# RKWin93/E2E-MAPPO-for-MT-FJSP

Measured on AMD Instinct MI355X. Metric: env-steps/sec (batched J6M6E2), higher is better.
Workload: dtype f64 (environment) / f32 (encoder: f32 storage and accumulation; 128x128 products on the 16-bit matrix cores from split f32 operands, f32-accurate: DESIGN.md §4)

## Files before the change

__graft_entry__.py:

```python
#!/usr/bin/env python3
import os
import sys

ROOT = os.path.dirname(os.path.abspath(__file__))
if ROOT not in sys.path:
    sys.path.insert(0, ROOT)


def build() -> None:
    from importlib import import_module
    import mtfjsp_amd
    _build = import_module("e2e-mappo-for-mt-fjsp_amd._build")
    lib = _build.build(force=True, verbose=True)
    capi = import_module("e2e-mappo-for-mt-fjsp_amd.capi")
    capi.lib()
    print("variant:", _build.build_variant("funcs", ["-DMTFJSP_BODY_FUNCS=3"]))
    from oracle import env_oracle
    print("oracle:", env_oracle.build(force=True))
    print("built", lib)


def smoke() -> None:
    import numpy as np
    import torch
    from importlib import import_module
    import mtfjsp_amd
    assert torch.cuda.is_available(), "smoke() needs cuda:0"
    batch_env = import_module("e2e-mappo-for-mt-fjsp_amd.batch_env")
    inst = import_module("e2e-mappo-for-mt-fjsp_amd.instances")
    from oracle.env_oracle import OracleBatch
    J, M, E, B = 6, 6, 2, 8
    T = J * M
    t, p, tt, edge = inst.generate_instances(B, J, M, E, seed=0)
    import random
    random.seed(0)
    w3 = inst.random_weights(B)
    env = batch_env.DeviceBatchEnv(J, M, E, B, obs_dtype="f64")
    env.load_instances(t, p, tt, edge=edge)
    env.scaler_init()
    env.reset(w3)
    orc = OracleBatch(t, p, tt, edge)
    orc.scaler_init()
    orc.reset(w3)
    a = torch.zeros(B, dtype=torch.int32, device=env.device); m = torch.zeros_like(a); j = torch.zeros_like(a)
    for s in range(T):
        env.random_actions(7, s, a, m, j)
        env.step(a, m)
        info, raw, _ = orc.step(a.cpu().numpy(), m.cpu().numpy())
        cand, mask = orc.job_mask_update(j.cpu().numpy())
        o = orc.observe()
        assert np.array_equal(env.info.cpu().numpy(), info), f"step {s}: rewards differ"
        assert np.array_equal(env.tasks_fea.cpu().numpy(), o["tfea"]), f"step {s}: tasks_fea differ"
        assert np.array_equal(env.dense_adj().cpu().numpy(), o["adj"]), f"step {s}: adj differ"
        assert np.array_equal(env.m_fea2.cpu().numpy(), o["mfea2"])
        assert np.array_equal(env.candidate.cpu().numpy(), cand) and np.array_equal(env.job_mask.cpu().numpy(), mask)
    assert bool(env.info[:, 1].all())
    _smoke_encoder()
    print("smoke OK: HIP env == oracle on", B, "instances x", T, "steps")


def _smoke_encoder() -> None:
    try:
        from importlib import import_module
        enc = import_module("e2e-mappo-for-mt-fjsp_amd.encoder")
    except ImportError:
        return
    if hasattr(enc, "smoke"):
        enc.smoke()


if __name__ == "__main__":
    cmd = sys.argv[1] if len(sys.argv) > 1 else "build"
    {"build": build, "smoke": smoke}[cmd]()
```

e2e-mappo-for-mt-fjsp_amd/csrc/mtfjsp_encoder.hip:

```cpp
#include <hip/hip_runtime.h>
#include <math.h>
#include <stdint.h>
#include <stdio.h>
#include <stdlib.h>
#include <string.h>
#include <algorithm>
#include <map>
#include <stdexcept>
#include <string>
#include <vector>

#include "../../include/mtfjsp.h"


#include "mtfjsp_enc_shared.h"

enum { PRO_PLAIN = 0, PRO_BNRELU = 1, PRO_AGG = 2, PRO_GIN0 = 3, PRO_GIN0BN = 4 };
enum { EPI_PLAIN = 0, EPI_STATS = 1, EPI_TANH = 2 };

struct GemmArgs {
    const float *in;
    int N;
    const float *Wt;
    const void *Wx6;
// ... 1279 lines not shown
__device__ __forceinline__ float pick_uniform(int b, uint64_t seed, uint64_t counter)
{
    uint32_t c[4] = {(uint32_t)b, (uint32_t)counter, (uint32_t)(counter >> 32), 0x73616d70u};
    philox4x32(c, (uint32_t)seed, (uint32_t)(seed >> 32));
    return (float)(c[0] >> 8) * (1.0f / 16777216.0f);
}
__device__ __forceinline__ int pick_action_u(const float *p, int n, int greedy, float u)
{
    int pick = 0;
    if (greedy) {
        float best = p[0];
        for (int i = 1; i < n; i++) if (p[i] > best) { best = p[i]; pick = i; }
    } else {
        float tot = 0.f;
        for (int i = 0; i < n; i++) tot += p[i];
        float acc = 0.f;
        const float thr = u * tot;
        pick = -1;
        int last = 0;
        for (int i = 0; i < n; i++) {
            if (p[i] > 0.f) {
                last = i;
                acc += p[i];
                if (pick < 0 && thr < acc) pick = i;
            }
        }
        if (pick < 0) pick = last;
    }
    return pick;
}
__device__ __forceinline__ int pick_action(const float *p, int n, int b, int greedy, uint64_t seed, uint64_t counter)
{
    int pick = 0;
    if (greedy) {
        float best = p[0];
        for (int i = 1; i < n; i++) if (p[i] > best) { best = p[i]; pick = i; }
    } else {
        uint32_t c[4] = {(uint32_t)b, (uint32_t)counter, (uint32_t)(counter >> 32), 0x73616d70u};
        philox4x32(c, (uint32_t)seed, (uint32_t)(seed >> 32));
        const float u = (float)(c[0] >> 8) * (1.0f / 16777216.0f);
        float tot = 0.f;
        for (int i = 0; i < n; i++) tot += p[i];
        float acc = 0.f;
        const float thr = u * tot;
        pick = -1;
        int last = 0;
        for (int i = 0; i < n; i++) {
            if (p[i] > 0.f) {
                last = i;
                acc += p[i];
                if (pick < 0 && thr < acc) pick = i;
            }
        }
        if (pick < 0) pick = last;
    }
    return pick;
}

struct HeadArgs {
    int B, R;
    int hg;
    const float *X;
    const float *pooled, *other;
    const float *W0i;
    const float *b0, *W1i, *b1, *w2, *b2;
    const float *Wc0i, *bc0, *Wc1i, *bc1, *wc2, *bc2;
    const void *W0x, *W1x, *Wc0x, *Wc1x;
    float sW0, sW1, sWc0, sWc1;
    const uint8_t *mask;
    float scale;
    float *prob, *value;
    const double *xbn_stats; const float *xbn_gamma, *xbn_beta; double xbn_inv_rows; float *pooled_out;
    const int *xgather; int xT, xrelu;
    int sample_mode; unsigned long long seed, counter; int *idx_out; float *logp_out; const int *gather_from; int *gathered_out;
    mtfjsp_mfea1_ctx_t mf; int mf_on;
    double *zero_stats; int zero_count;
    double *zero_stats2; int zero_count2;
    unsigned long long *stamps;
    unsigned *range_flag;
};
#define HG 16
#define HCH 6
#define HX_NPART 32

__global__ __launch_bounds__(512) void k_heads(HeadArgs A)
{
    extern __shared__ __align__(16) unsigned char smem[];
    float *s_x = reinterpret_cast<float *>(smem);
    float *s_s = s_x + HCH * 16 * LDA16;
    float *s_p = s_s + HCH * 16 * LDA16;
    float *s_o = s_p + 16 * LDA16;
    float *s_c1 = s_o + 16 * LDA16;
    float *s_c2 = s_c1 + 16 * LDA16;
    float *s_u = s_c2 + 16 * LDA16;
    float *s_part = s_u + HG * HD;
    float *s_score = s_part + 8 * HCH * 16;
    float *s_wc2 = s_score + HG * 64;
    unsigned char *s_mask = reinterpret_cast<unsigned char *>(s_wc2 + 2 * HD);
    const int tid = threadIdx.x, wave = tid >> 6, lane = tid & 63;
    const int m = lane & 15, q = lane >> 4;
    const int col = 16 * wave + m;
#ifdef MTFJSP_STAMP
    unsigned long long ph[8] = {0, 0, 0, 0, 0, 0, 0, 0}, t_last;
    asm volatile("s_memtime %0\n\ts_waitcnt lgkmcnt(0)" : "=s"(t_last)::"memory");
#endif
    const int R = A.R;
    const unsigned invR = (unsigned)((0x100000000ull + (unsigned)R - 1) / (unsigned)R);
#define WCOL(dst, Wi)                                                                              \
    do {                                                                                           \
        const float4 *w_ = reinterpret_cast<const float4 *>(Wi) + (size_t)wave * 8 * 64 + lane;    \
        _Pragma("unroll") for (int g_ = 0; g_ < 8; g_++) {                                         \
            const float4 v_ = w_[g_ * 64];                                                         \
            dst[4 * g_] = v_.x; dst[4 * g_ + 1] = v_.y; dst[4 * g_ + 2] = v_.z; dst[4 * g_ + 3] = v_.w; \
        }                                                                                          \
    } while (0)
#define TILE2(acc0, acc1, t0p, t1p, bw)                                                                          \
    do {                                                                                                         \
        _Pragma("unroll") for (int s_ = 0; s_ < 32; s_++) {                                                      \
            acc0 = __builtin_amdgcn_mfma_f32_16x16x4f32((t0p)[4 * s_], bw[s_], acc0, 0, 0, 0);                   \
            acc1 = __builtin_amdgcn_mfma_f32_16x16x4f32((t1p)[4 * s_], bw[s_], acc1, 0, 0, 0);                   \
        }                                                                                                        \
        MFMA_SETTLE2(acc0, acc1);                                                                                \
    } while (0)
    const int sr = tid >> 5, sc4 = (tid & 31) * 4;
    const int aoff = m * LDA16 + q;
    const float b0c = A.b0[col], bc0c = A.bc0[col], bc1c = A.bc1[col], b1c = A.b1[col], w2c = A.w2[col], b2 = A.b2[0];
    if (tid < 2 * HD) s_wc2[tid] = A.wc2[tid];
    const f32x4 zero4 = {0.f, 0.f, 0.f, 0.f};
    if (A.zero_stats && blockIdx.x == 0) for (int i = tid; i < A.zero_count; i += 512) A.zero_stats[i] = 0.0;
    if (A.zero_stats2 && blockIdx.x == 0) for (int i = tid; i < A.zero_count2; i += 512) A.zero_stats2[i] = 0.0;
    float xs0 = 1.f, xs1 = 1.f, xs2 = 1.f, xs3 = 1.f, xh0 = 0.f, xh1 = 0.f, xh2 = 0.f, xh3 = 0.f;
    if (A.xbn_stats) {
        stage_bn(s_u, A.xbn_stats, A.xbn_inv_rows, A.xbn_gamma, A.xbn_beta, tid);
        LDS_BARRIER();
        xs0 = s_u[sc4]; xs1 = s_u[sc4 + 1]; xs2 = s_u[sc4 + 2]; xs3 = s_u[sc4 + 3];
        xh0 = s_u[HD + sc4]; xh1 = s_u[HD + sc4 + 1]; xh2 = s_u[HD + sc4 + 2]; xh3 = s_u[HD + sc4 + 3];
        LDS_BARRIER();
    }
    STAMP(6);
    {
        const int g0 = blockIdx.x * HG;
        const int ng = (A.B - g0) < HG ? (A.B - g0) : HG;
        const int nrows = ng * R;
        float wA[32], wB[32], wC[32];
        WCOL(wA, A.W0i + 1 * HD * HD);
        WCOL(wB, A.W0i + 2 * HD * HD);
        WCOL(wC, A.Wc0i);
        {
            const float4 z = make_float4(0.f, 0.f, 0.f, 0.f);
            float4 xp = z;
            if (A.xbn_stats) {
                if (sr < ng) {
                    const int nr = A.xgather ? A.xT : R;
                    const float *src = A.X + (size_t)(g0 + sr) * nr * HD + sc4;
                    float a0 = 0.f, a1 = 0.f, a2 = 0.f, a3 = 0.f;
#pragma unroll 12
                    for (int r = 0; r < nr; r++) {
                        const float4 v = *reinterpret_cast<const float4 *>(src + (size_t)r * HD);
                        float y0 = fmaf(v.x, xs0, xh0), y1 = fmaf(v.y, xs1, xh1), y2 = fmaf(v.z, xs2, xh2), y3 = fmaf(v.w, xs3, xh3);
                        if (A.xrelu) { y0 = fmaxf(y0, 0.f); y1 = fmaxf(y1, 0.f); y2 = fmaxf(y2, 0.f); y3 = fmaxf(y3, 0.f); }
                        a0 += y0; a1 += y1; a2 += y2; a3 += y3;
                    }
                    const float ir = 1.0f / (float)nr;
                    xp = make_float4(a0 * ir, a1 * ir, a2 * ir, a3 * ir);
                    *reinterpret_cast<float4 *>(A.pooled_out + (size_t)(g0 + sr) * HD + sc4) = xp;
                }
// ... 103 lines not shown
                if (part == 0 && r < ng) { A.value[(size_t)(g0 + r) * 2] = p0 + A.bc2[0]; A.value[(size_t)(g0 + r) * 2 + 1] = p1 + A.bc2[1]; }
            }
            LDS_BARRIER();
            if (tid < nt * 16) {
                const int grow = tb * 16 + tid;
                float v = b2;
                for (int w = 0; w < 8; w++) v += s_part[w * (HCH * 16) + tid];
                if (grow < nrows) s_score[grow] = v * A.scale;
            }
            LDS_BARRIER();
            STAMP(4);
        }
        {
            const int r0 = tid >> 4, l = tid & 15;
            if (r0 < ng) {
                float mx = -INFINITY;
                for (int r = l; r < R; r += 16) if (!s_mask[r0 * R + r]) mx = fmaxf(mx, s_score[r0 * R + r]);
                for (int o = 8; o > 0; o >>= 1) mx = fmaxf(mx, __shfl_xor(mx, o));
                float sum = 0.f;
                for (int r = l; r < R; r += 16) if (!s_mask[r0 * R + r]) sum += __expf(s_score[r0 * R + r] - mx);
                for (int o = 8; o > 0; o >>= 1) sum += __shfl_xor(sum, o);
                for (int r = l; r < R; r += 16) {
                    const float pr = s_mask[r0 * R + r] ? 0.f : __expf(s_score[r0 * R + r] - mx) / sum;
                    A.prob[(size_t)(g0 + r0) * R + r] = pr;
                    s_score[r0 * R + r] = pr;
                }
                if (A.sample_mode) {
                    asm volatile("s_waitcnt lgkmcnt(0)" ::: "memory");
                    if (l == 0) {
                        const int b = g0 + r0;
                        const int pick = pick_action(s_score + r0 * R, R, b, A.sample_mode == 2, A.seed, A.counter);
                        A.idx_out[b] = pick;
                        if (A.logp_out) A.logp_out[b] = logf(s_score[r0 * R + pick]);
                        const int gsel = A.gather_from ? A.gather_from[(size_t)b * R + pick] : pick;
                        if (A.gather_from && A.gathered_out) A.gathered_out[b] = gsel;
                        s_part[r0] = __int_as_float(gsel);
                    }
                    if (A.mf_on) {
                        asm volatile("s_waitcnt lgkmcnt(0)" ::: "memory");
                        const int b = g0 + r0, T_ = A.mf.T, M_ = A.mf.M;
                        int a = __float_as_int(s_part[r0]);
                        if (a < 0 || a >= T_) a = 0;
                        const size_t row = (size_t)b * T_ + a;
                        int pm = 0;
                        if (a % M_ != 0) {
                            pm = reinterpret_cast<const short *>(A.mf.link)[(row - 1) * 8 + 4];
                            if (pm < 0) pm += M_;
                        }
                        for (int mm = l; mm < M_; mm += 16) {
                            const double tv = A.mf.t[row * M_ + mm], pv = A.mf.p[row * M_ + mm];
                            const double ptv = tv * fabs(pv);
                            const unsigned char mk = (unsigned char)!(tv >= 0);
                            const double x = (a % M_ != 0) ? A.mf.tt[((size_t)b * M_ + pm) * M_ + mm] : 0.0;
                            const double f0 = tv > 0 ? tv : A.mf.mean3[row * 3 + 0], f1 = ptv > 0 ? ptv : A.mf.mean3[row * 3 + 1];
                            const double f4 = pv > 0 ? pv : A.mf.mean3[row * 3 + 2];
                            const size_t o = ((size_t)b * M_ + mm) * 6;
                            const double f3 = (double)(1 - (int)mk), f5 = (double)(A.mf.shop[(size_t)b * M_ + mm] + 1);
                            if (A.mf.obs_f32) {
                                float *of = reinterpret_cast<float *>(A.mf.m_fea1_out) + o;
                                of[0] = (float)f0; of[1] = (float)f1; of[2] = (float)x; of[3] = (float)f3; of[4] = (float)f4; of[5] = (float)f5;
                            } else {
                                double *od = reinterpret_cast<double *>(A.mf.m_fea1_out) + o;
                                od[0] = f0; od[1] = f1; od[2] = x; od[3] = f3; od[4] = f4; od[5] = f5;
                            }
                            A.mf.mmask_out[(size_t)b * M_ + mm] = mk;
                        }
                    }
                }
            }
        }
        STAMP(5);
    }
#ifdef MTFJSP_STAMP
    if (A.stamps && lane == 0) for (int i = 0; i < 8; i++) A.stamps[((size_t)blockIdx.x * 8 + wave) * 8 + i] = ph[i];
#endif
}
static size_t heads_lds_bytes() { return (size_t)((2 * HCH + 4) * 16 * LDA16 + HG * HD + 8 * HCH * 16 + HG * 64 + 2 * HD) * 4 + HG * 64; }

#define WCOLX(dst, Wx, blk)                                                                                     \
    do {                                                                                                         \
        const float4 *w_ = reinterpret_cast<const float4 *>(Wx) + ((size_t)(blk) * 8 + wave) * (2 * 4 * 64) + lane; \
        _Pragma("unroll") for (int p_ = 0; p_ < 2; p_++)                                                         \
            _Pragma("unroll") for (int k_ = 0; k_ < 4; k_++) dst[p_][k_] = __builtin_bit_cast(h16x8, w_[(p_ * 4 + k_) * 64]); \
    } while (0)
#define X6_STEP(accA, accB, wv, xv, ks)                                                          \
    do {                                                                                          \
        accB = __builtin_amdgcn_mfma_f32_16x16x32_f16(wv[0][ks], xv[1], accB, 0, 0, 0);           \
        accA = __builtin_amdgcn_mfma_f32_16x16x32_f16(wv[0][ks], xv[0], accA, 0, 0, 0);           \
        accB = __builtin_amdgcn_mfma_f32_16x16x32_f16(wv[1][ks], xv[0], accB, 0, 0, 0);           \
    } while (0)
#define HX_CLDA 132
#if MTFJSP_BODY_FUNCS & 2
__device__ __forceinline__ void headsx_body(const HeadArgs &A, unsigned char *smem)
{
#include "mtfjsp_headsx_body.h"
}
#endif
__global__ __launch_bounds__(512) void k_headsx(HeadArgs A)
{
    extern __shared__ __align__(16) unsigned char smem[];
#if MTFJSP_BODY_FUNCS & 2
    headsx_body(A, smem);
#else
#include "mtfjsp_headsx_body.h"
#endif
}
__global__ __launch_bounds__(512) void k_headsx_gat3x(HeadArgs HA, GatArgs GA)
{
    extern __shared__ __align__(16) unsigned char smem[];
#if MTFJSP_BODY_FUNCS & 2
    headsx_body(HA, smem);
#else
    {
        const HeadArgs &A = HA;
#include "mtfjsp_headsx_body.h"
    }
#endif
    __syncthreads();
#if MTFJSP_BODY_FUNCS & 1
    gat3x_body(GA, smem);
#else
    {
        const GatArgs &A = GA;
#include "mtfjsp_gat3x_body.h"
    }
#endif
}
#define GAT_IMG_OFF (128 * 1024)
#define GAT_IMG_BYTES (8 * 64 * 4 * 4 + 256 * 4)
#define GAT_F1_OFF (GAT_IMG_OFF + GAT_IMG_BYTES)
#define GAT_F2_OFF (GAT_F1_OFF + 16 * 8 * 6 * 4)
#define GAT_PRE_END (GAT_F2_OFF + 16 * 8 * 8 * 4)
__device__ __forceinline__ void gat_f2_load(const GatArgs &G, int t, int M, float (&x)[4])
{
    const size_t base = (size_t)blockIdx.x * 16 * M * 8, total = (size_t)G.R * 8;
#pragma unroll
    for (int i = 0; i < 4; i++) {
        const size_t idx = base + (size_t)(i * 256 + t), ic = idx < total ? idx : total - 1;
        x[i] = G.feat_f64 ? (float)reinterpret_cast<const double *>(G.f2)[ic] : reinterpret_cast<const float *>(G.f2)[ic];
        if (!(i * 256 + t < 16 * M * 8 && idx < total)) x[i] = 0.f;
    }
}
__device__ __forceinline__ void gat_prestage(const GatArgs &G, unsigned char *smem, int t, const float (&x)[4])
{
    const float4 *src = reinterpret_cast<const float4 *>(G.Wx6);
    float4 v[16];
#pragma unroll
    for (int i = 0; i < 16; i++) v[i] = src[i * 256 + t];
    const float4 q0 = reinterpret_cast<const float4 *>(G.Wq)[t], q1 = reinterpret_cast<const float4 *>(G.Wq)[256 + t];
    const float ga = G.gat_a[t];
    float4 *dst = reinterpret_cast<float4 *>(smem);
#pragma unroll
    for (int i = 0; i < 16; i++) dst[i * 256 + t] = v[i];
    float4 *img = reinterpret_cast<float4 *>(smem + GAT_IMG_OFF);
    img[t] = q0; img[256 + t] = q1;
    reinterpret_cast<float *>(smem + GAT_IMG_OFF + 8192)[t] = ga;
    float *d = reinterpret_cast<float *>(smem + GAT_F2_OFF);
#pragma unroll
    for (int i = 0; i < 4; i++) d[i * 256 + t] = x[i];
}
#if !MTFJSP_BODY_FUNCS
template <int ENV, bool NLDS>
__global__ __launch_bounds__(512) void k_headsx_gat3x_headsx(HeadArgs HA, GatArgs GA, HeadArgs HM, XchgArgs XG, EnvParams EP)
{
    extern __shared__ __align__(16) unsigned char smem[];
    const XchgArgs &XA = XG;
// ... 2366 lines not shown
```

e2e-mappo-for-mt-fjsp_amd/csrc/mtfjsp_headsx_body.h:

```cpp
#ifndef HX_NLDS
#define HX_NLDS false
#endif
#ifndef HX_VALUES_ONLY
#define HX_VALUES_ONLY 0
#endif
    unsigned char *s_xs = smem;
    unsigned char *s_pp = s_xs + HCH * X2_TILE;
    unsigned char *s_op = s_pp + X2_TILE;
    unsigned char *s_c1p = s_op + X2_TILE;
    float *s_c2 = reinterpret_cast<float *>(s_c1p + X2_TILE);
    float *s_u = s_c2 + 16 * HX_CLDA;
    float *s_part = s_u + HG * HD;
    float *s_score = s_part + HX_NPART * HCH * 16;
    float *s_wc2 = s_score + HG * 64;
    float *s_vec = s_wc2 + 2 * HD;
    unsigned char *s_mask = reinterpret_cast<unsigned char *>(s_vec + 5 * HD);
    int *s_gf = reinterpret_cast<int *>(s_mask + HG * 64);
    int *s_pm = s_gf + 512;
    const int tid = BODY_TID, wave = __builtin_amdgcn_readfirstlane(tid >> 6), lane = tid & 63;
    const int m = lane & 15, q = lane >> 4;
    const int col4 = 16 * wave + 4 * q;
#ifdef MTFJSP_STAMP
    unsigned long long ph[8] = {0, 0, 0, 0, 0, 0, 0, 0}, t_last;
    asm volatile("s_memtime %0\n\ts_waitcnt lgkmcnt(0)" : "=s"(t_last)::"memory");
#endif
    const int R = A.R;
    const unsigned invR = (unsigned)((0x100000000ull + (unsigned)R - 1) / (unsigned)R);
    const int sr = tid >> 5, sc4 = (tid & 31) * 4;
    const int xoff = m * X6_ROWB + 16 * q;
    const float b2 = A.b2[0];
    const float r_wc2 = A.wc2[tid & (2 * HD - 1)];
    const int tc = tid & (HD - 1);
    const float r_v0 = A.b0[tc], r_v1 = A.bc0[tc], r_v2 = A.bc1[tc], r_v3 = A.b1[tc], r_v4 = A.w2[tc];
    const f32x4 zero4 = {0.f, 0.f, 0.f, 0.f};
    float xs0 = 1.f, xs1 = 1.f, xs2 = 1.f, xs3 = 1.f, xh0 = 0.f, xh1 = 0.f, xh2 = 0.f, xh3 = 0.f;
    double bsu[STAT_REP], bsq[STAT_REP];
    float bga = 0.f, bbe = 0.f;
    if (A.xbn_stats) {
#if !HX_XCHG
#pragma unroll
        for (int r = 0; r < STAT_REP; r++) { bsu[r] = A.xbn_stats[r * 256 + tc]; bsq[r] = A.xbn_stats[r * 256 + HD + tc]; }
#endif
        bga = A.xbn_gamma[tc]; bbe = A.xbn_beta[tc];
    }
    {
        const int g0 = blockIdx.x * A.hg;
        const int ng = (A.B - g0) < A.hg ? (A.B - g0) : A.hg;
        const int nrows = ng * R;
        auto xrow = [&](int grow) __attribute__((always_inline)) -> const float * {
            if (!A.xgather) return A.X + ((size_t)g0 * R + grow) * HD + sc4;
            const int il = (int)__umulhi((unsigned)grow, invR);
            return A.X + ((size_t)(g0 + il) * A.xT + A.xgather[(size_t)g0 * R + grow]) * HD + sc4;
        };
#if HX_XCHG
        const bool by_inst = R <= HCH;
        float4 praw = make_float4(0.f, 0.f, 0.f, 0.f), xo_pre;
        xo_pre = *reinterpret_cast<const float4 *>(A.other + (size_t)(g0 + (sr < ng ? sr : ng - 1)) * HD + sc4);
        if (!by_inst) {
            const int ic = sr < ng ? sr : ng - 1;
            const float *src = A.X + (size_t)(g0 + ic) * R * HD + sc4;
            float4 rv[8];
#pragma unroll
            for (int r = 0; r < 8; r++) rv[r] = *reinterpret_cast<const float4 *>(src + (size_t)(r < R ? r : R - 1) * HD);
            const float ir = 1.0f / (float)R;
#pragma unroll
            for (int r = 0; r < 8; r++) {
                const float wgt = r < R ? ir : 0.f;
                praw.x = fmaf(rv[r].x, wgt, praw.x); praw.y = fmaf(rv[r].y, wgt, praw.y); praw.z = fmaf(rv[r].z, wgt, praw.z); praw.w = fmaf(rv[r].w, wgt, praw.w);
            }
            asm volatile("" : "+v"(praw.x), "+v"(praw.y), "+v"(praw.z), "+v"(praw.w));
        }
#else
        const bool by_inst = false;
#endif
        const unsigned char r_mask = A.mask[(size_t)g0 * R + (tid < nrows ? tid : nrows - 1)];
#if !HX_XCHG
        const float4 xp_top = *reinterpret_cast<const float4 *>((A.pooled ? A.pooled : A.other) + (size_t)(g0 + (sr < ng ? sr : ng - 1)) * HD + sc4);
        const float4 xo_top = *reinterpret_cast<const float4 *>(A.other + (size_t)(g0 + (sr < ng ? sr : ng - 1)) * HD + sc4);
#endif
        const int r_gf = (A.gather_from ? A.gather_from + (size_t)g0 * R : reinterpret_cast<const int *>(A.X))[tid < nrows ? tid : nrows - 1];
        h16x8 wA[2][4], wB[2][4], wC[2][4];
        const float sW0 = A.sW0, sW1 = A.sW1, sWc0 = A.sWc0, sWc1 = A.sWc1;
        WCOLX(wA, A.W0x, 1);
        WCOLX(wB, A.W0x, 2);
        WCOLX(wC, A.Wc0x, 0);
        float4 xr[HCH];
        if (HX_VALUES_ONLY) { for (int t = 0; t < HCH; t++) xr[t] = make_float4(0.f, 0.f, 0.f, 0.f); }
        else {
            int gi[HCH];
#pragma unroll
            for (int t = 0; t < HCH; t++) {
                const int grow = by_inst ? sr * R + t : t * 16 + sr, gc = (grow < nrows && (!by_inst || t < R)) ? grow : nrows - 1;
                gi[t] = A.xgather ? A.xgather[(size_t)g0 * R + gc] : gc;
            }
#pragma unroll
            for (int t = 0; t < HCH; t++) {
                const int grow = by_inst ? sr * R + t : t * 16 + sr, gc = (grow < nrows && (!by_inst || t < R)) ? grow : nrows - 1;
                const int il = (int)__umulhi((unsigned)gc, invR);
                if (HX_NLDS) {
                    xr[t] = *reinterpret_cast<const float4 *>(reinterpret_cast<const float *>(smem + 8 * 2 * 4 * 64 * 16) + ((gc >> 3) * 16 + (gc & 7)) * HD + sc4);
                    continue;
                }
                const float *src = A.xgather ? A.X + ((size_t)(g0 + il) * A.xT + gi[t]) * HD + sc4 : A.X + ((size_t)g0 * R + gc) * HD + sc4;
                xr[t] = *reinterpret_cast<const float4 *>(src);
// ... 81 lines not shown
        }
        STAMP(6); H3_RT(6);
        {
            const float4 z = make_float4(0.f, 0.f, 0.f, 0.f);
            float4 xp = z;
#if HX_XCHG
            if (by_inst) {
                const float ir = 1.0f / (float)R;
#pragma unroll
                for (int t = 0; t < HCH; t++) {
                    const float wgt = t < R ? ir : 0.f;
                    praw.x = fmaf(xr[t].x, wgt, praw.x); praw.y = fmaf(xr[t].y, wgt, praw.y); praw.z = fmaf(xr[t].z, wgt, praw.z); praw.w = fmaf(xr[t].w, wgt, praw.w);
                }
            }
            if (sr < ng) {
                xp = make_float4(fmaf(praw.x, xs0, xh0), fmaf(praw.y, xs1, xh1), fmaf(praw.z, xs2, xh2), fmaf(praw.w, xs3, xh3));
                *reinterpret_cast<float4 *>(A.pooled_out + (size_t)(g0 + sr) * HD + sc4) = xp;
            }
#else
            if (A.xbn_stats) {
                if (sr < ng) {
                    const int nr = A.xgather ? A.xT : R;
                    const float *src = A.X + (size_t)(g0 + sr) * nr * HD + sc4;
                    float a0 = 0.f, a1 = 0.f, a2 = 0.f, a3 = 0.f;
#pragma unroll 12
                    for (int r = 0; r < nr; r++) {
                        const float4 v = *reinterpret_cast<const float4 *>(src + (size_t)r * HD);
                        float y0 = fmaf(v.x, xs0, xh0), y1 = fmaf(v.y, xs1, xh1), y2 = fmaf(v.z, xs2, xh2), y3 = fmaf(v.w, xs3, xh3);
                        if (A.xrelu) { y0 = fmaxf(y0, 0.f); y1 = fmaxf(y1, 0.f); y2 = fmaxf(y2, 0.f); y3 = fmaxf(y3, 0.f); }
                        a0 += y0; a1 += y1; a2 += y2; a3 += y3;
                    }
                    const float ir = 1.0f / (float)nr;
                    xp = make_float4(a0 * ir, a1 * ir, a2 * ir, a3 * ir);
                    *reinterpret_cast<float4 *>(A.pooled_out + (size_t)(g0 + sr) * HD + sc4) = xp;
                }
            } else if (sr < ng) xp = xp_top;
#endif
            STAMP(7); H3_RT(7);
#if HX_XCHG
            const float4 xo = sr < ng ? xo_pre : z;
#else
            const float4 xo = sr < ng ? xo_top : z;
#endif
            {
                const float vp[4] = {xp.x, xp.y, xp.z, xp.w}, vo[4] = {xo.x, xo.y, xo.z, xo.w};
                uint2 a0, a1, b0, b1;
                split2x4(vp, a0, a1); split2x4(vo, b0, b1);
                unsigned char *dp = s_pp + sr * X6_ROWB + (tid & 31) * 8, *dq = s_op + sr * X6_ROWB + (tid & 31) * 8;
                *reinterpret_cast<uint2 *>(dp) = a0; *reinterpret_cast<uint2 *>(dp + X6_PLANE) = a1;
                *reinterpret_cast<uint2 *>(dq) = b0; *reinterpret_cast<uint2 *>(dq + X6_PLANE) = b1;
            }
        }
        if (tid < nrows) s_mask[tid] = r_mask;
        short r_lk;
        {
            const int T_ = A.mf_on ? A.mf.T : 1, il = (int)__umulhi((unsigned)(tid < nrows ? tid : 0), invR);
            int a = A.gather_from ? r_gf : 0;
            if (a < 0 || a >= T_) a = 0;
            const size_t row = (size_t)(g0 + il) * T_ + a;
            r_lk = (A.mf_on ? reinterpret_cast<const short *>(A.mf.link) : reinterpret_cast<const short *>(A.X))[(A.mf_on && row > 0 ? row - 1 : 0) * 8 + 4];
            s_gf[tid] = r_gf;
        }
        for (int i = tid + 512; i < nrows; i += 512) s_mask[i] = A.mask[(size_t)g0 * R + i];
        LDS_BARRIER();
        STAMP(0); H3_RT(0);
        auto xnorm = [&](float4 v, bool valid) __attribute__((always_inline)) {
            if (!valid) return make_float4(0.f, 0.f, 0.f, 0.f);
            float y0 = fmaf(v.x, xs0, xh0), y1 = fmaf(v.y, xs1, xh1), y2 = fmaf(v.z, xs2, xh2), y3 = fmaf(v.w, xs3, xh3);
            if (A.xrelu) { y0 = fmaxf(y0, 0.f); y1 = fmaxf(y1, 0.f); y2 = fmaxf(y2, 0.f); y3 = fmaxf(y3, 0.f); }
            return make_float4(y0, y1, y2, y3);
        };
        auto tile_x6 = [&](const unsigned char *tp, const h16x8 (&wv)[2][4]) __attribute__((always_inline)) -> f32x4 {
            f32x4 aA = zero4, aB = zero4;
            h16x8 xv[4][2];
#pragma unroll
            for (int ks = 0; ks < 4; ks++)
#pragma unroll
                for (int p = 0; p < 2; p++) xv[ks][p] = *reinterpret_cast<const h16x8 *>(tp + xoff + p * X6_PLANE + 64 * ks);
#pragma unroll
            for (int ks = 0; ks < 4; ks++) X6_STEP(aA, aB, wv, xv[ks], ks);
            MFMA_SETTLE2(aA, aB);
            return aA + aB;
        };
        auto put_planes = [&](unsigned char *tp, const float (&v)[4]) __attribute__((always_inline)) {
            uint2 p0, p1;
            split2x4(v, p0, p1);
            unsigned char *d = tp + m * X6_ROWB + col4 * 2;
            *reinterpret_cast<uint2 *>(d) = p0; *reinterpret_cast<uint2 *>(d + X6_PLANE) = p1;
        };
        {
            const f32x4 au = tile_x6(s_pp, wA) + tile_x6(s_op, wB);
            const f32x4 ac = tile_x6(s_pp, wC);
            WCOLX(wA, A.Wc1x, 0);
            WCOLX(wB, A.W0x, 0);
            WCOLX(wC, A.W1x, 0);
            const float4 b0v = *reinterpret_cast<const float4 *>(s_vec + col4), bc0v = *reinterpret_cast<const float4 *>(s_vec + HD + col4);
            *reinterpret_cast<float4 *>(s_u + m * HD + col4) = make_float4(fmaf(au[0], sW0, b0v.x), fmaf(au[1], sW0, b0v.y), fmaf(au[2], sW0, b0v.z), fmaf(au[3], sW0, b0v.w));
            const float c1v[4] = {fast_tanh(fmaf(ac[0], sWc0, bc0v.x)), fast_tanh(fmaf(ac[1], sWc0, bc0v.y)), fast_tanh(fmaf(ac[2], sWc0, bc0v.z)), fast_tanh(fmaf(ac[3], sWc0, bc0v.w))};
            put_planes(s_c1p, c1v);
        }
        s_pm[tid] = (int)r_lk;
        STAMP(1); H3_RT(1);
#if HX_VALUES_ONLY
        {
            LDS_BARRIER();
            const f32x4 a0 = tile_x6(s_c1p, wA);
            const float4 bc1v = *reinterpret_cast<const float4 *>(s_vec + 2 * HD + col4);
            *reinterpret_cast<float4 *>(s_c2 + m * HX_CLDA + col4) =
                make_float4(fast_tanh(fmaf(a0[0], sWc1, bc1v.x)), fast_tanh(fmaf(a0[1], sWc1, bc1v.y)), fast_tanh(fmaf(a0[2], sWc1, bc1v.z)), fast_tanh(fmaf(a0[3], sWc1, bc1v.w)));
            LDS_BARRIER();
            if (tid < 256) {
                const int r = tid >> 4, part = tid & 15;
                float p0 = 0.f, p1 = 0.f;
                const float4 xa_ = *reinterpret_cast<const float4 *>(s_c2 + r * HX_CLDA + part * 8), xb_ = *reinterpret_cast<const float4 *>(s_c2 + r * HX_CLDA + part * 8 + 4);
                const float4 wa0 = *reinterpret_cast<const float4 *>(s_wc2 + part * 8), wb0 = *reinterpret_cast<const float4 *>(s_wc2 + part * 8 + 4);
                const float4 wa1 = *reinterpret_cast<const float4 *>(s_wc2 + HD + part * 8), wb1 = *reinterpret_cast<const float4 *>(s_wc2 + HD + part * 8 + 4);
                const float xs[8] = {xa_.x, xa_.y, xa_.z, xa_.w, xb_.x, xb_.y, xb_.z, xb_.w};
                const float w0s[8] = {wa0.x, wa0.y, wa0.z, wa0.w, wb0.x, wb0.y, wb0.z, wb0.w}, w1s[8] = {wa1.x, wa1.y, wa1.z, wa1.w, wb1.x, wb1.y, wb1.z, wb1.w};
#pragma unroll
                for (int k = 0; k < 8; k++) { p0 = fmaf(xs[k], w0s[k], p0); p1 = fmaf(xs[k], w1s[k], p1); }
                p0 = row_sum16(p0); p1 = row_sum16(p1);
                if (part == 0 && r < ng) {
                    const float v0 = p0 + A.bc2[0], v1 = p1 + A.bc2[1];
                    A.value[(size_t)(g0 + r) * 2] = v0; A.value[(size_t)(g0 + r) * 2 + 1] = v1;
                    if (A.range_flag && (v0 != v0 || v1 != v1)) __hip_atomic_store(A.range_flag, 1u, __ATOMIC_RELAXED, __HIP_MEMORY_SCOPE_SYSTEM);
                }
            }
            (void)xnorm; (void)b2; (void)invR; (void)xoff;
        }
#else
        const int ntl = (nrows + 15) >> 4;
        for (int tb = 0; tb < ntl; tb += HCH) {
            const int nt = (ntl - tb) < HCH ? (ntl - tb) : HCH;
#pragma unroll
            for (int t = 0; t < HCH; t++) {
                if (tb > 0) {
                    const int grow = (tb + t) * 16 + sr;
                    xr[t] = (tb + t < ntl && grow < nrows) ? *reinterpret_cast<const float4 *>(xrow(grow)) : make_float4(0.f, 0.f, 0.f, 0.f);
                }
                const int srow = by_inst ? sr * R + t : (tb + t) * 16 + sr;
                const float4 xv4 = xnorm(xr[t], srow < nrows);
                const float v[4] = {xv4.x, xv4.y, xv4.z, xv4.w};
                uint2 p0, p1;
                split2x4(v, p0, p1);
                unsigned char *d = by_inst ? s_xs + (srow >> 4) * X2_TILE + (srow & 15) * X6_ROWB + (tid & 31) * 8 : s_xs + t * X2_TILE + sr * X6_ROWB + (tid & 31) * 8;
                if (!by_inst || t < R) { *reinterpret_cast<uint2 *>(d) = p0; *reinterpret_cast<uint2 *>(d + X6_PLANE) = p1; }
            }
            LDS_BARRIER();
            STAMP(2); H3_RT(2);
            f32x4 accb[HCH];
#pragma unroll
            for (int t = 0; t < HCH; t++) accb[t] = t < nt ? tile_x6(s_xs + t * X2_TILE, wB) : zero4;
            H3S_RT(0);
            if (tb == 0) {
                const f32x4 a0 = tile_x6(s_c1p, wA);
                const float4 bc1v = *reinterpret_cast<const float4 *>(s_vec + 2 * HD + col4);
                *reinterpret_cast<float4 *>(s_c2 + m * HX_CLDA + col4) =
                    make_float4(fast_tanh(fmaf(a0[0], sWc1, bc1v.x)), fast_tanh(fmaf(a0[1], sWc1, bc1v.y)), fast_tanh(fmaf(a0[2], sWc1, bc1v.z)), fast_tanh(fmaf(a0[3], sWc1, bc1v.w)));
            }
            H3S_RT(1);
            LDS_BARRIER();
            H3S_RT(2);
#pragma unroll
            for (int t = 0; t < HCH; t++) {
                if (t < nt) {
                    const int grow = (tb + t) * 16 + m;
                    const int i0 = grow < nrows ? (int)__umulhi((unsigned)grow, invR) : 0;
                    const float4 uv = *reinterpret_cast<const float4 *>(s_u + i0 * HD + col4);
                    const float sv[4] = {fast_tanh(fmaf(accb[t][0], sW0, uv.x)), fast_tanh(fmaf(accb[t][1], sW0, uv.y)), fast_tanh(fmaf(accb[t][2], sW0, uv.z)), fast_tanh(fmaf(accb[t][3], sW0, uv.w))};
                    put_planes(s_xs + t * X2_TILE, sv);
                }
            }
            H3S_RT(3);
            LDS_BARRIER();
            STAMP(3); H3_RT(3);
            {
                const float4 b1v = *reinterpret_cast<const float4 *>(s_vec + 3 * HD + col4), w2v = *reinterpret_cast<const float4 *>(s_vec + 4 * HD + col4);
#pragma unroll 1
                for (int t = 0; t < HCH; t++) {
                    if (t < nt) {
                        const f32x4 a0 = tile_x6(s_xs + t * X2_TILE, wC);
                        float v = fast_tanh(fmaf(a0[0], sW1, b1v.x)) * w2v.x;
                        v = fmaf(fast_tanh(fmaf(a0[1], sW1, b1v.y)), w2v.y, v);
                        v = fmaf(fast_tanh(fmaf(a0[2], sW1, b1v.z)), w2v.z, v);
                        v = fmaf(fast_tanh(fmaf(a0[3], sW1, b1v.w)), w2v.w, v);
#if HX_NPART == 32
                        s_part[(wave * 4 + q) * (HCH * 16) + t * 16 + m] = v;
#else
                        v += __shfl_xor(v, 16);
                        v += __shfl_xor(v, 32);
                        if (q == 0) s_part[wave * (HCH * 16) + t * 16 + m] = v;
#endif
                    }
                }
            }
            H3S_RT(4);
            if (tb == 0 && tid < 256) {
                const int r = tid >> 4, part = tid & 15;
                float p0 = 0.f, p1 = 0.f;
                const float4 xa_ = *reinterpret_cast<const float4 *>(s_c2 + r * HX_CLDA + part * 8), xb_ = *reinterpret_cast<const float4 *>(s_c2 + r * HX_CLDA + part * 8 + 4);
                const float4 wa0 = *reinterpret_cast<const float4 *>(s_wc2 + part * 8), wb0 = *reinterpret_cast<const float4 *>(s_wc2 + part * 8 + 4);
                const float4 wa1 = *reinterpret_cast<const float4 *>(s_wc2 + HD + part * 8), wb1 = *reinterpret_cast<const float4 *>(s_wc2 + HD + part * 8 + 4);
                const float xs[8] = {xa_.x, xa_.y, xa_.z, xa_.w, xb_.x, xb_.y, xb_.z, xb_.w};
                const float w0s[8] = {wa0.x, wa0.y, wa0.z, wa0.w, wb0.x, wb0.y, wb0.z, wb0.w}, w1s[8] = {wa1.x, wa1.y, wa1.z, wa1.w, wb1.x, wb1.y, wb1.z, wb1.w};
#pragma unroll
                for (int k = 0; k < 8; k++) { p0 = fmaf(xs[k], w0s[k], p0); p1 = fmaf(xs[k], w1s[k], p1); }
                p0 = row_sum16(p0); p1 = row_sum16(p1);
                if (part == 0 && r < ng) {
                    const float v0 = p0 + A.bc2[0], v1 = p1 + A.bc2[1];
                    A.value[(size_t)(g0 + r) * 2] = v0; A.value[(size_t)(g0 + r) * 2 + 1] = v1;
                    if (A.range_flag && (v0 != v0 || v1 != v1)) __hip_atomic_store(A.range_flag, 1u, __ATOMIC_RELAXED, __HIP_MEMORY_SCOPE_SYSTEM);
                }
            }
            H3S_RT(5);
            LDS_BARRIER();
            if (tid < nt * 16) {
                const int grow = tb * 16 + tid;
                float v = b2;
#pragma unroll
                for (int w = 0; w < HX_NPART; w++) v += s_part[w * (HCH * 16) + tid];
                if (grow < nrows) s_score[grow] = v * A.scale;
            }
            H3S_RT(6);
            LDS_BARRIER();
            STAMP(4); H3_RT(4);
        }
#if HX_XCHG
        X3_RT(6);
#endif
#ifdef HX_IDLE_HOOK
        if (tid >= 256) { HX_IDLE_HOOK }
#endif
        {
            const int r0 = tid >> 4, l = tid & 15;
            const bool rowwise = R <= 16;
            float pr_l = 0.f;
            int pick_l = 0;
            if (r0 < ng && rowwise) {
                auto dpp = [&](float x, auto Ctrl) __attribute__((always_inline)) {
                    return __builtin_bit_cast(float, __builtin_amdgcn_update_dpp(0, __builtin_bit_cast(int, x), decltype(Ctrl)::value, 0xF, 0xF, true));
                };
                auto x8 = [&](float x) __attribute__((always_inline)) { return dpp(x, std::integral_constant<int, 0x128>{}); };
                auto x4 = [&](float x) __attribute__((always_inline)) {
                    const float up = dpp(x, std::integral_constant<int, 0x12C>{}), dn = dpp(x, std::integral_constant<int, 0x124>{});
                    return (l & 4) ? dn : up;
                };
                auto x2 = [&](float x) __attribute__((always_inline)) { return dpp(x, std::integral_constant<int, 0x4E>{}); };
                auto x1 = [&](float x) __attribute__((always_inline)) { return dpp(x, std::integral_constant<int, 0xB1>{}); };
                const bool on = l < R && !s_mask[r0 * R + (l < R ? l : 0)];
                const float sc = s_score[r0 * R + (l < R ? l : 0)];
                float mx = on ? sc : -INFINITY;
                mx = fmaxf(mx, x8(mx)); mx = fmaxf(mx, x4(mx)); mx = fmaxf(mx, x2(mx)); mx = fmaxf(mx, x1(mx));
                const float ex = on ? __expf(sc - mx) : 0.f;
                float sum = ex;
                sum += x8(sum); sum += x4(sum); sum += x2(sum); sum += x1(sum);
                pr_l = on ? ex / sum : 0.f;
                if (l < R) {
                    A.prob[(size_t)(g0 + r0) * R + l] = pr_l;
                    if (A.range_flag && pr_l != pr_l) __hip_atomic_store(A.range_flag, 1u, __ATOMIC_RELAXED, __HIP_MEMORY_SCOPE_SYSTEM);
                }
                H3S_RT(7);
                if (A.sample_mode) {
                    float run = pr_l;
#pragma unroll 1
                    for (int k = 1; k < R; k++) {
                        const float prev = dpp(run, std::integral_constant<int, 0x111>{});
                        if (l == k) run = prev + pr_l;
                    }
                    const float tot = __shfl(run, (lane & 48) + R - 1);
                    const float thr = u_pre * tot;
                    const bool pos = l < R && pr_l > 0.f;
                    const unsigned hit = (unsigned)(__builtin_amdgcn_ballot_w64(pos && thr < run) >> (lane & 48)) & 0xffffu;
                    const unsigned any = (unsigned)(__builtin_amdgcn_ballot_w64(pos) >> (lane & 48)) & 0xffffu;
                    pick_l = hit ? __builtin_ctz(hit) : any ? 31 - __builtin_clz(any) : 0;
                    if (A.sample_mode == 2) {
                        float best = l < R ? pr_l : -INFINITY;
                        best = fmaxf(best, x8(best)); best = fmaxf(best, x4(best)); best = fmaxf(best, x2(best)); best = fmaxf(best, x1(best));
                        const unsigned eq = (unsigned)(__builtin_amdgcn_ballot_w64(l < R && pr_l == best) >> (lane & 48)) & 0xffffu;
// ... 93 lines not shown
```

Before: 20.68 million.

## Pair waves over 32-column blocks in heads kernel to halve LDS activation reads

New measurement: 20.28 million. -1.9%, worse.

```diff
diff --git a/__graft_entry__.py b/__graft_entry__.py
--- a/__graft_entry__.py
+++ b/__graft_entry__.py
@@ -15,6 +15,7 @@
     capi = import_module("e2e-mappo-for-mt-fjsp_amd.capi")
     capi.lib()
     print("variant:", _build.build_variant("funcs", ["-DMTFJSP_BODY_FUNCS=3"]))
+    print("variant:", _build.build_variant("wcols16", ["-DHX_WAVE_COLS=16"]))
     from oracle import env_oracle
     print("oracle:", env_oracle.build(force=True))
     print("built", lib)
diff --git a/e2e-mappo-for-mt-fjsp_amd/csrc/mtfjsp_encoder.hip b/e2e-mappo-for-mt-fjsp_amd/csrc/mtfjsp_encoder.hip
--- a/e2e-mappo-for-mt-fjsp_amd/csrc/mtfjsp_encoder.hip
+++ b/e2e-mappo-for-mt-fjsp_amd/csrc/mtfjsp_encoder.hip
@@ -1385,6 +1385,13 @@
 #define HG 16
 #define HCH 6
 #define HX_NPART 32
+#ifndef HX_WAVE_COLS
+#define HX_WAVE_COLS 32
+#endif
+#define HX_PAIR (HX_WAVE_COLS == 32 && HX_NPART == 32 && !HX_VALUES_ONLY && !HX_ABL)
+#ifndef HX_ABL
+#define HX_ABL 0
+#endif
 
 __global__ __launch_bounds__(512) void k_heads(HeadArgs A)
 {
@@ -1654,6 +1661,14 @@
         const float4 *w_ = reinterpret_cast<const float4 *>(Wx) + ((size_t)(blk) * 8 + wave) * (2 * 4 * 64) + lane; \
         _Pragma("unroll") for (int p_ = 0; p_ < 2; p_++)                                                         \
             _Pragma("unroll") for (int k_ = 0; k_ < 4; k_++) dst[p_][k_] = __builtin_bit_cast(h16x8, w_[(p_ * 4 + k_) * 64]); \
+    } while (0)
+#define WCOLX2(dst0, dst1, Wx, blk, cblk, ln)                                                                    \
+    do {                                                                                                         \
+        const float4 *w_ = reinterpret_cast<const float4 *>(Wx) + ((size_t)(blk) * 8 + (cblk)) * (2 * 4 * 64) + (ln); \
+        _Pragma("unroll") for (int p_ = 0; p_ < 2; p_++)                                                         \
+            _Pragma("unroll") for (int k_ = 0; k_ < 4; k_++) dst0[p_][k_] = __builtin_bit_cast(h16x8, w_[(p_ * 4 + k_) * 64]); \
+        _Pragma("unroll") for (int p_ = 0; p_ < 2; p_++)                                                         \
+            _Pragma("unroll") for (int k_ = 0; k_ < 4; k_++) dst1[p_][k_] = __builtin_bit_cast(h16x8, w_[(8 + p_ * 4 + k_) * 64]); \
     } while (0)
 #define X6_STEP(accA, accB, wv, xv, ks)                                                          \
     do {                                                                                          \
diff --git a/e2e-mappo-for-mt-fjsp_amd/csrc/mtfjsp_headsx_body.h b/e2e-mappo-for-mt-fjsp_amd/csrc/mtfjsp_headsx_body.h
--- a/e2e-mappo-for-mt-fjsp_amd/csrc/mtfjsp_headsx_body.h
+++ b/e2e-mappo-for-mt-fjsp_amd/csrc/mtfjsp_headsx_body.h
@@ -20,6 +20,10 @@
     const int tid = BODY_TID, wave = __builtin_amdgcn_readfirstlane(tid >> 6), lane = tid & 63;
     const int m = lane & 15, q = lane >> 4;
     const int col4 = 16 * wave + 4 * q;
+#if HX_PAIR
+    const int cb = wave & 3, par = wave >> 2;
+    const int colp[2] = {32 * cb + 4 * q, 32 * cb + 16 + 4 * q};
+#endif
 #ifdef MTFJSP_STAMP
     unsigned long long ph[8] = {0, 0, 0, 0, 0, 0, 0, 0}, t_last;
     asm volatile("s_memtime %0\n\ts_waitcnt lgkmcnt(0)" : "=s"(t_last)::"memory");
@@ -267,22 +271,56 @@
             MFMA_SETTLE2(aA, aB);
             return aA + aB;
         };
-        auto put_planes = [&](unsigned char *tp, const float (&v)[4]) __attribute__((always_inline)) {
+#if HX_PAIR
+        auto tile_x6p = [&](const unsigned char *tp, const h16x8 (&wv0)[2][4], const h16x8 (&wv1)[2][4], f32x4 &r0, f32x4 &r1) __attribute__((always_inline)) {
+            f32x4 aA = zero4, aB = zero4, bA = zero4, bB = zero4;
+            h16x8 xv[4][2];
+#pragma unroll
+            for (int ks = 0; ks < 4; ks++)
+#pragma unroll
+                for (int p = 0; p < 2; p++) xv[ks][p] = *reinterpret_cast<const h16x8 *>(tp + xoff + p * X6_PLANE + 64 * ks);
+#pragma unroll
+            for (int ks = 0; ks < 4; ks++) { X6_STEP(aA, aB, wv0, xv[ks], ks); X6_STEP(bA, bB, wv1, xv[ks], ks); }
+            MFMA_SETTLE2(aA, aB); MFMA_SETTLE2(bA, bB);
+            r0 = aA + aB; r1 = bA + bB;
+        };
+#endif
+#if HX_ABL & 1
+        h16x8 xabl[4][2];
+        auto tile_x6abl = [&](const unsigned char *tp, const h16x8 (&wv)[2][4], bool read) __attribute__((always_inline)) -> f32x4 {
+            f32x4 aA = zero4, aB = zero4;
+            if (read) {
+#pragma unroll
+                for (int ks = 0; ks < 4; ks++)
+#pragma unroll
+                    for (int p = 0; p < 2; p++) xabl[ks][p] = *reinterpret_cast<const h16x8 *>(tp + xoff + p * X6_PLANE + 64 * ks);
+            }
+#pragma unroll
+            for (int ks = 0; ks < 4; ks++) X6_STEP(aA, aB, wv, xabl[ks], ks);
+            MFMA_SETTLE2(aA, aB);
+            return aA + aB;
+        };
+#endif
+        auto put_planes = [&](unsigned char *tp, const float (&v)[4], int c4) __attribute__((always_inline)) {
             uint2 p0, p1;
             split2x4(v, p0, p1);
-            unsigned char *d = tp + m * X6_ROWB + col4 * 2;
+            unsigned char *d = tp + m * X6_ROWB + c4 * 2;
             *reinterpret_cast<uint2 *>(d) = p0; *reinterpret_cast<uint2 *>(d + X6_PLANE) = p1;
         };
         {
             const f32x4 au = tile_x6(s_pp, wA) + tile_x6(s_op, wB);
             const f32x4 ac = tile_x6(s_pp, wC);
             WCOLX(wA, A.Wc1x, 0);
+#if HX_PAIR
+            WCOLX2(wB, wC, A.W0x, 0, 2 * cb, lane);
+#else
             WCOLX(wB, A.W0x, 0);
             WCOLX(wC, A.W1x, 0);
+#endif
             const float4 b0v = *reinterpret_cast<const float4 *>(s_vec + col4), bc0v = *reinterpret_cast<const float4 *>(s_vec + HD + col4);
             *reinterpret_cast<float4 *>(s_u + m * HD + col4) = make_float4(fmaf(au[0], sW0, b0v.x), fmaf(au[1], sW0, b0v.y), fmaf(au[2], sW0, b0v.z), fmaf(au[3], sW0, b0v.w));
             const float c1v[4] = {fast_tanh(fmaf(ac[0], sWc0, bc0v.x)), fast_tanh(fmaf(ac[1], sWc0, bc0v.y)), fast_tanh(fmaf(ac[2], sWc0, bc0v.z)), fast_tanh(fmaf(ac[3], sWc0, bc0v.w))};
-            put_planes(s_c1p, c1v);
+            put_planes(s_c1p, c1v, col4);
         }
         s_pm[tid] = (int)r_lk;
         STAMP(1); H3_RT(1);
@@ -317,6 +355,11 @@
         const int ntl = (nrows + 15) >> 4;
         for (int tb = 0; tb < ntl; tb += HCH) {
             const int nt = (ntl - tb) < HCH ? (ntl - tb) : HCH;
+#if HX_PAIR
+            int ln = lane;
+            asm volatile("" : "+v"(ln));
+            if (tb > 0) WCOLX2(wB, wC, A.W0x, 0, 2 * cb, ln);
+#endif
 #pragma unroll
             for (int t = 0; t < HCH; t++) {
                 if (tb > 0) {
@@ -333,19 +376,51 @@
             }
             LDS_BARRIER();
             STAMP(2); H3_RT(2);
-            f32x4 accb[HCH];
-#pragma unroll
-            for (int t = 0; t < HCH; t++) accb[t] = t < nt ? tile_x6(s_xs + t * X2_TILE, wB) : zero4;
-            H3S_RT(0);
-            if (tb == 0) {
+            auto c2_tile = [&]() __attribute__((always_inline)) {
                 const f32x4 a0 = tile_x6(s_c1p, wA);
                 const float4 bc1v = *reinterpret_cast<const float4 *>(s_vec + 2 * HD + col4);
                 *reinterpret_cast<float4 *>(s_c2 + m * HX_CLDA + col4) =
                     make_float4(fast_tanh(fmaf(a0[0], sWc1, bc1v.x)), fast_tanh(fmaf(a0[1], sWc1, bc1v.y)), fast_tanh(fmaf(a0[2], sWc1, bc1v.z)), fast_tanh(fmaf(a0[3], sWc1, bc1v.w)));
-            }
+            };
+#if HX_PAIR
+            f32x4 accb[HCH / 2][2];
+#pragma unroll
+            for (int j = 0; j < HCH / 2; j++) {
+                const int t = 2 * j + par;
+                accb[j][0] = accb[j][1] = zero4;
+                if (t < nt) tile_x6p(s_xs + t * X2_TILE, wB, wC, accb[j][0], accb[j][1]);
+            }
+            WCOLX2(wB, wC, A.W1x, 0, 2 * cb, ln);
+#elif HX_ABL & 1
+            f32x4 accb[HCH];
+#pragma unroll
+            for (int t = 0; t < HCH; t++) accb[t] = t < nt ? tile_x6abl(s_xs + t * X2_TILE, wB, !(t & 1)) : zero4;
+#else
+            f32x4 accb[HCH];
+#pragma unroll
+            for (int t = 0; t < HCH; t++) accb[t] = t < nt ? tile_x6(s_xs + t * X2_TILE, wB) : zero4;
+#endif
+            H3S_RT(0);
+            if (tb == 0) c2_tile();
             H3S_RT(1);
             LDS_BARRIER();
             H3S_RT(2);
+#if HX_PAIR
+#pragma unroll
+            for (int j = 0; j < HCH / 2; j++) {
+                const int t = 2 * j + par;
+                if (t < nt) {
+                    const int grow = (tb + t) * 16 + m;
+                    const int i0 = grow < nrows ? (int)__umulhi((unsigned)grow, invR) : 0;
+#pragma unroll
+                    for (int h = 0; h < 2; h++) {
+                        const float4 uv = *reinterpret_cast<const float4 *>(s_u + i0 * HD + colp[h]);
+                        const float sv[4] = {fast_tanh(fmaf(accb[j][h][0], sW0, uv.x)), fast_tanh(fmaf(accb[j][h][1], sW0, uv.y)), fast_tanh(fmaf(accb[j][h][2], sW0, uv.z)), fast_tanh(fmaf(accb[j][h][3], sW0, uv.w))};
+                        put_planes(s_xs + t * X2_TILE, sv, colp[h]);
+                    }
+                }
+            }
+#else
 #pragma unroll
             for (int t = 0; t < HCH; t++) {
                 if (t < nt) {
@@ -353,18 +428,46 @@
                     const int i0 = grow < nrows ? (int)__umulhi((unsigned)grow, invR) : 0;
                     const float4 uv = *reinterpret_cast<const float4 *>(s_u + i0 * HD + col4);
                     const float sv[4] = {fast_tanh(fmaf(accb[t][0], sW0, uv.x)), fast_tanh(fmaf(accb[t][1], sW0, uv.y)), fast_tanh(fmaf(accb[t][2], sW0, uv.z)), fast_tanh(fmaf(accb[t][3], sW0, uv.w))};
-                    put_planes(s_xs + t * X2_TILE, sv);
-                }
-            }
+                    put_planes(s_xs + t * X2_TILE, sv, col4);
+                }
+            }
+#endif
             H3S_RT(3);
             LDS_BARRIER();
             STAMP(3); H3_RT(3);
+#if HX_PAIR
+            {
+                float4 b1v[2], w2v[2];
+#pragma unroll
+                for (int h = 0; h < 2; h++) { b1v[h] = *reinterpret_cast<const float4 *>(s_vec + 3 * HD + colp[h]); w2v[h] = *reinterpret_cast<const float4 *>(s_vec + 4 * HD + colp[h]); }
+#pragma unroll 1
+                for (int j = 0; j < HCH / 2; j++) {
+                    const int t = 2 * j + par;
+                    if (t < nt) {
+                        f32x4 a[2];
+                        tile_x6p(s_xs + t * X2_TILE, wB, wC, a[0], a[1]);
+#pragma unroll
+                        for (int h = 0; h < 2; h++) {
+                            float v = fast_tanh(fmaf(a[h][0], sW1, b1v[h].x)) * w2v[h].x;
+                            v = fmaf(fast_tanh(fmaf(a[h][1], sW1, b1v[h].y)), w2v[h].y, v);
+                            v = fmaf(fast_tanh(fmaf(a[h][2], sW1, b1v[h].z)), w2v[h].z, v);
+                            v = fmaf(fast_tanh(fmaf(a[h][3], sW1, b1v[h].w)), w2v[h].w, v);
+                            s_part[((2 * cb + h) * 4 + q) * (HCH * 16) + t * 16 + m] = v;
+                        }
+                    }
+                }
+            }
+#else
             {
                 const float4 b1v = *reinterpret_cast<const float4 *>(s_vec + 3 * HD + col4), w2v = *reinterpret_cast<const float4 *>(s_vec + 4 * HD + col4);
 #pragma unroll 1
                 for (int t = 0; t < HCH; t++) {
                     if (t < nt) {
+#if HX_ABL & 1
+                        const f32x4 a0 = tile_x6abl(s_xs + t * X2_TILE, wC, !(t & 1));
+#else
                         const f32x4 a0 = tile_x6(s_xs + t * X2_TILE, wC);
+#endif
                         float v = fast_tanh(fmaf(a0[0], sW1, b1v.x)) * w2v.x;
                         v = fmaf(fast_tanh(fmaf(a0[1], sW1, b1v.y)), w2v.y, v);
                         v = fmaf(fast_tanh(fmaf(a0[2], sW1, b1v.z)), w2v.z, v);
@@ -379,6 +482,7 @@
                     }
                 }
             }
+#endif
             H3S_RT(4);
             if (tb == 0 && tid < 256) {
                 const int r = tid >> 4, part = tid & 15;
```
